# PANXIONG-CN/TEC-MoLLM

Hardware: AMD Instinct MI355X
Metric: train samples/sec (higher is better)
Workload: dtype f32; 1 GPU; BASELINE configs[1]: B=8/GPU, L_in=48, L_out=12, N=2911, F=10 (d_emb=12), 3 GPT-2 blocks, full fwd+bwd+AdamW, fp32, GATv2 per_timestep, dropout on (p=0.1); global_batch=8, parallelism=dp1, data_feed=fixed, launch=eager

## Files before the change

include/tecmollm.h:

```cpp
#ifndef TECMOLLM_H
#define TECMOLLM_H

#include <stdint.h>

#ifdef __cplusplus
extern "C" {
#endif

#define TECM_OK 0
#define TECM_E_ARG (-1)
#define TECM_E_ALIGN (-2)
#define TECM_E_LAUNCH (-3)
#define TECM_E_LDS (-4)

#define TECM_ABI_VERSION 17
int tecm_abi_version(void);
const char* tecm_last_error(void);

typedef struct TecmWin {
  int32_t enabled;
  int32_t N;
  int32_t Lin, Lout;
  int32_t stride_t;
  int32_t taps;
// ... 116 lines not shown
typedef struct TecmLnDyMap {
  int32_t T, N;
  TecmDrop drop;
} TecmLnDyMap;
int tecm_layernorm_bwd(const float* dy, int64_t lddy, const float* x, int64_t ldx, const float* gamma,
                       const float* stats, const float* dres, float* dx, void* dx_masked, int32_t masked_bf16,
                       const TecmDrop* mask_drop, float* dgb_partials, int32_t* num_blocks, int64_t M, int32_t D,
                       const TecmLnAdd* add ,
                       int32_t dy_bf16 ,
                       const TecmLnDyMap* dymap , void* stream);

#define TECM_ATT_OUT_BF16 1
#define TECM_ATT_QKV_BF16 2
#define TECM_ATT_DCTX_BF16 4
int tecm_attention_fwd(const float* qkv, void* ctx, int32_t io_bf16, int32_t B, int32_t T, int32_t N, int32_t heads,
                       int32_t D, const TecmDrop* prob_drop, void* stream);
int tecm_attention_bwd(const float* qkv, const float* dctx, void* dqkv, int32_t io_bf16, int32_t B, int32_t T, int32_t N,
                       int32_t heads, int32_t D, const TecmDrop* prob_drop, void* stream);

int tecm_colsum(const float* in, int64_t ld, int64_t outer, int64_t inner, int32_t nseg, int32_t C,
                float* out, int64_t ldo, int32_t accumulate, float scale, const TecmDrop* in_drop,
                float* workspace , void* stream);
int tecm_colsum_twin(const float* in, int64_t ld, int64_t outer, int64_t inner, int32_t nseg, int32_t C,
                     float* out, int64_t ldo, int32_t accumulate, float scale, const TecmDrop* in_drop,
                     float* workspace, void* twin_bf16, int64_t ld_twin, void* stream);

int tecm_huber_fwd_bwd(const float* pred, const float* target, float* dpred, float* loss_out,
                       int64_t n, float delta, float grad_scale, float* workspace ,
                       void* stream);

int tecm_conv_weight_pack(const float* w, float* fwd_pack, float* bwd_pack, int32_t Cout, int32_t Cin,
                          int32_t k, void* stream);
int tecm_conv_weight_unpack(const float* dpack, float* dw, int32_t Cout, int32_t Cin, int32_t k,
                            void* stream);

typedef struct TecmConvDx {
  const void* dy;
  const void* wpack;
  float* dinp;
  int32_t B, Lc, N, Cout, ld_in, _pad;
} TecmConvDx;
int tecm_conv_dx_pack(const float* w3, const float* w5, const float* w7, void* wpack, int32_t Cout, int32_t Cin,
                      int32_t ld_in, void* stream);
int tecm_conv_dx_bf16(const TecmConvDx* p, void* stream);
typedef struct TecmConvFwd {
  const void* inp;
  const void* wpack;
  const float* bias;
  float* y;
  int32_t B, Lc, N, Cout, ld_in, y_bf16;
  float* stats;
  float eps;
  int32_t _pad;
} TecmConvFwd;
int tecm_conv_fwd_pack(const float* w3, const float* w5, const float* w7, void* wpack, int32_t Cout, int32_t Cin,
                       int32_t ld_in, void* stream);
int tecm_conv_fwd_bf16(const TecmConvFwd* p, void* stream);
int tecm_conv_fwd_pack_f32(const float* w3, const float* w5, const float* w7, float* wpack, int32_t Cout, int32_t Cin,
                           int32_t ld_in, void* stream);
int tecm_conv_fwd_f32(const TecmConvFwd* p, void* stream);
int tecm_conv_dx_pack_f32(const float* w3, const float* w5, const float* w7, float* wpack, int32_t Cout, int32_t Cin,
                          int32_t ld_in, void* stream);
int tecm_conv_dx_f32(const TecmConvDx* p, void* stream);
int tecm_conv_fwd_supported(int32_t Lc, int32_t Cout, int32_t ld_in, int32_t f32);
int tecm_conv_dx_supported(int32_t Lc, int32_t Cout, int32_t ld_in, int32_t f32);

typedef struct TecmConvDw {
  const void* inp;
  const void* dy;
  float* workspace;
  float* dw3;
  float* dw5;
  float* dw7;
  int32_t B, Lc, N, Cout, Cin, ld_in, num_blocks, _pad;
} TecmConvDw;
int tecm_huber_fwd_bwd_strided(const float* pred, const int64_t* pred_strides , const float* target,
                               const int64_t* target_strides , float* dpred, float* loss_out, int32_t B, int32_t H,
                               int32_t N, float delta, float grad_scale, float* workspace , void* stream);

int64_t tecm_conv_dw_workspace(int32_t Cout, int32_t ld_in, int32_t num_blocks);
int tecm_conv_dw_bf16(const TecmConvDw* p, void* stream);
int tecm_conv_dw_f32(const TecmConvDw* p, void* stream);

int tecm_cast_bf16(const float* src, int64_t ld_src, void* dst, int64_t ld_dst, int64_t rows, int32_t cols, void* stream);

int tecm_weight_bf16(const float* src, int64_t ld_src, void* same_bf16, int64_t ld_same, void* transposed_bf16, int64_t ld_tr,
                     int32_t rows, int32_t cols, void* stream);

int tecm_dropout_apply(const float* src, int64_t ld_src, void* dst, int64_t ld_dst, int32_t dst_bf16, void* dst2_bf16,
                       int64_t ld_dst2, int64_t rows, int32_t cols, const TecmDrop* drop, void* stream);

int tecm_transpose_scale(const float* src, int64_t lds, float* dst, int64_t ldd, int32_t rows,
                         int32_t cols, float scale, void* stream);

int tecm_lora_fold(const float* lora_B, int32_t n_out, int32_t r, float scale, void* w_kn, int64_t ld_kn, int32_t kn_bf16,
                   void* w_nk, int64_t ld_nk, int32_t nk_bf16, int32_t k_off, void* stream);

int tecm_pack_vectors(const float* const* srcs, const int32_t* lens, int32_t count, float* dst, void* stream);

#define TECM_NORM_BLOCKS 512
typedef struct {
  int64_t n;
  float* param; float* grad; float* exp_avg; float* exp_avg_sq;
  double* partials;
  float* total_norm_out;
  float lr, beta1, beta2, eps, weight_decay, max_norm, grad_scale;
// ... 35 lines not shown
```

tec-mollm_amd/csrc/conv_seq.hip:

```cpp
#include "common.h"
#include <type_traits>

typedef float f32x16 __attribute__((ext_vector_type(16)));
typedef __bf16 bf16x8 __attribute__((ext_vector_type(8)));
typedef unsigned int u32x4 __attribute__((ext_vector_type(4)));
typedef float f32x4 __attribute__((ext_vector_type(4)));

namespace tecm_convseq {

#ifndef CDX_ABLATE
#define CDX_ABLATE 0
#endif

constexpr int NB = 4;
constexpr int NTH = 256;
constexpr int MAXT = 6;

__host__ __device__ __forceinline__ int seg_nact(int d) {
  const int a = d < 3 ? 3 - d : d - 3;
  return a <= 1 ? 3 : (a == 2 ? 2 : 1);
}

struct Args {
  const void* dy;
// ... 325 lines not shown
    while (k >= seg_nact(d) * Cout) {
      k -= seg_nact(d) * Cout;
      ++d;
    }
    const int col = (3 - seg_nact(d)) * Cout + k;
    const int j = col / Cout, co = col - j * Cout;
    const int kj = 3 + 2 * j, tau = (kj - 1) / 2 - (d - 3);
    const float* w = j == 0 ? w3 : (j == 1 ? w5 : w7);
    float v = 0.f;
    if (ci < Cin && tau >= 0 && tau < kj) v = w[((int64_t)co * Cin + ci) * kj + tau];
    wpack[i] = (__bf16)v;
  }
}

}

namespace tecm_convseq {

__device__ __forceinline__ float wave_total_dpp(float v) {
  auto step = [](float x, auto ctrl, auto rmask) {
    constexpr int C = decltype(ctrl)::value, R = decltype(rmask)::value;
    return x + __builtin_bit_cast(float, __builtin_amdgcn_update_dpp(0, __builtin_bit_cast(int, x), C, R, 0xF, false));
  };
  v = step(v, std::integral_constant<int, 0xB1>{}, std::integral_constant<int, 0xF>{});
  v = step(v, std::integral_constant<int, 0x4E>{}, std::integral_constant<int, 0xF>{});
  v = step(v, std::integral_constant<int, 0x141>{}, std::integral_constant<int, 0xF>{});
  v = step(v, std::integral_constant<int, 0x140>{}, std::integral_constant<int, 0xF>{});
  v = step(v, std::integral_constant<int, 0x142>{}, std::integral_constant<int, 0xA>{});
  v = step(v, std::integral_constant<int, 0x143>{}, std::integral_constant<int, 0xC>{});
  return __builtin_bit_cast(float, __builtin_amdgcn_readlane(__builtin_bit_cast(int, v), 63));
}

constexpr int FMAXU = 12;
#ifndef CFW_PD
#define CFW_PD 4
#endif
#ifndef CFW_ABLATE
#define CFW_ABLATE 0
#endif
#ifndef CFW_PD32
#define CFW_PD32 1
#endif
struct FArgs {
  const void* inp;
  const void* wpack;
  const float* bias;
  float* y;
  int y16;
  float* stats;
  float eps;
  int B, Lc, N, Cout, ld_in, TC, nchunk, nblk, pitch;
  int nb32;
  unsigned long long assign;
};

#ifdef CFW_STAMPS
__device__ unsigned long long cfw_stamps[16 * 8192];
}
extern "C" int tecm_cfw_stamps_read(unsigned long long* dst, int n) {
  return (int)hipMemcpyFromSymbol(dst, HIP_SYMBOL(tecm_convseq::cfw_stamps), sizeof(unsigned long long) * n);
}
namespace tecm_convseq {
#define CFW_STAMP(i) do { if (threadIdx.x == 0 && blockIdx.x < 8192) cfw_stamps[blockIdx.x * 16 + (i)] = __builtin_amdgcn_s_memrealtime(); } while (0)
#else
#define CFW_STAMP(i) do { } while (0)
#endif
__global__ __launch_bounds__(NTH, 3) void conv_fwd_seq_kernel(const FArgs a) {
  extern __shared__ __attribute__((aligned(16))) unsigned char lds[];
  CFW_STAMP(0);
  const int tid = threadIdx.x, lane = tid & 63;
  const int wave = __builtin_amdgcn_readfirstlane(tid >> 6);
  const int r = lane & 31, h = lane >> 5;
  int tile = blockIdx.x;
  const int nbk = tile % a.nblk;
  tile /= a.nblk;
  const int chunk = tile % a.nchunk, b = tile / a.nchunk;
  const int n0 = nbk * NB, t0 = chunk * a.TC;
  const int tc = min(a.TC, a.Lc - t0);
  const int steps = tc + 7;
  const int CT = 3 * a.Cout;

  {
    const int cpr = a.ld_in / 8;
    const int total = steps * NB * cpr;
    for (int idx = tid; idx < total; idx += NTH) {
      const int row = idx / cpr, ch = idx - row * cpr;
      const int ts = t0 - 3 + (row >> 2);
      const int ng = min(n0 + (row & 3), a.N - 1);
      u32x4 v = {0u, 0u, 0u, 0u};
      if (!(CFW_ABLATE & 1) && ts >= 0 && ts < a.Lc)
        v = *reinterpret_cast<const u32x4*>(static_cast<const __bf16*>(a.inp) + (((int64_t)b * a.Lc + ts) * a.N + ng) * a.ld_in + ch * 8);
      *reinterpret_cast<u32x4*>(lds + row * a.pitch + ch * 16) = v;
    }
  }
  __syncthreads();
  CFW_STAMP(1);

  const int ntt = tc >> 3;
  const int cpt = a.ld_in / 8;
  const unsigned cpt_magic = (unsigned)((65536 + cpt - 1) / cpt);
  __shared__ float xst[4][3][2 * NB + 1];
  if (a.stats && lane < 3) xst[wave][lane][0] = -1.f;
#pragma unroll 1
  for (int ui = 0; ui < 3; ++ui) {
    const int u = (int)((a.assign >> (12 * wave + 4 * ui)) & 15ull);
    if (u == 15) break;
// ... 97 lines not shown
              s1[e & 3] += dv;
              s2[e & 3] += dv * dv;
            }
          }
        const float ucnt = (float)(32 * tc);
#pragma unroll
        for (int n = 0; n < NB; ++n) {
          const float t1 = wave_total_dpp(s1[n]), t2 = wave_total_dpp(s2[n]);
          if (lane == 0) {
            xst[wave][ui][1 + n] = sh + t1 / ucnt;
            xst[wave][ui][1 + NB + n] = fmaxf(t2 - t1 * t1 / ucnt, 0.f);
          }
        }
        if (lane == 0) xst[wave][ui][0] = (float)j;
      }
      continue;
    }
    float* yb = a.y + (((int64_t)b * a.Lc + t0 + h) * a.N + n0) * CT + col0 + r;
#pragma unroll
    for (int i = 0; i < MAXT; ++i) {
      if (i < ntt) {
#pragma unroll
        for (int e = 0; e < 16; ++e) {
          const int n = e & 3;
          if (n0 + n < a.N) yb[(8 * i + 2 * (e >> 2)) * tstride + n * CT] = acc[i][e] + bv;
        }
      }
    }
  }
  CFW_STAMP(8);
  if (a.stats) {
    __syncthreads();
    if (tid < 3 * NB) {
      const int jb = tid / NB, n = tid % NB;
      const float ucnt = (float)(32 * tc);
      float cnt = 0.f, mean = 0.f, m2 = 0.f;
      for (int w = 0; w < 4; ++w)
        for (int q = 0; q < 3; ++q)
          if (xst[w][q][0] == (float)jb) {
            const float tot = cnt + ucnt, fr = ucnt / tot, dl = xst[w][q][1 + n] - mean;
            m2 += xst[w][q][1 + NB + n] + dl * dl * cnt * fr;
            mean += dl * fr;
            cnt = tot;
          }
      if (n0 + n < a.N) {
        float* st = a.stats + (((int64_t)b * a.N + n0 + n) * 3 + jb) * 2;
        st[0] = mean;
        st[1] = 1.0f / sqrtf(m2 / cnt + a.eps);
      }
    }
  }
}

__global__ __launch_bounds__(NTH, 2) void conv_fwd_seq_f32_kernel(const FArgs a) {
  extern __shared__ __attribute__((aligned(16))) unsigned char lds[];
  const int tid = threadIdx.x, lane = tid & 63;
  const int wave = __builtin_amdgcn_readfirstlane(tid >> 6);
  const int r = lane & 31, h = lane >> 5;
  int tile = blockIdx.x;
  const int nbk = tile % a.nblk;
  tile /= a.nblk;
  const int chunk = tile % a.nchunk, b = tile / a.nchunk;
  const int n0 = nbk * NB, t0 = chunk * a.TC;
  const int tc = min(a.TC, a.Lc - t0);
  const int steps = tc + 7;
  const int CT = 3 * a.Cout;
  {
    const int cpr = a.ld_in / 4;
    const int total = steps * NB * cpr;
    const float* src = static_cast<const float*>(a.inp);
    for (int idx = tid; idx < total; idx += NTH) {
      const int row = idx / cpr, ch = idx - row * cpr;
      const int ts = t0 - 3 + (row >> 2);
      const int ng = min(n0 + (row & 3), a.N - 1);
      u32x4 v = {0u, 0u, 0u, 0u};
      if (ts >= 0 && ts < a.Lc)
        v = *reinterpret_cast<const u32x4*>(src + (((int64_t)b * a.Lc + ts) * a.N + ng) * a.ld_in + ch * 4);
      *reinterpret_cast<u32x4*>(lds + row * a.pitch + ch * 16) = v;
    }
  }
  __syncthreads();

  const int ntt = tc >> 3;
  const int cpt = a.ld_in / 4;
  const unsigned cpt_magic = (unsigned)((65536 + cpt - 1) / cpt);
#pragma unroll 1
  for (int ui = 0; ui < 3; ++ui) {
    const int u = (int)((a.assign >> (12 * wave + 4 * ui)) & 15ull);
    if (u == 15) break;
    const int j = u / a.nb32, kb = u - j * a.nb32;
    const int pad = j + 1, col0 = j * a.Cout + 32 * kb;
    const int st3 = 3 * a.ld_in / 8, st5 = 5 * a.ld_in / 8, st7 = 7 * a.ld_in / 8;
    const int nsteps = j == 0 ? st3 : (j == 1 ? st5 : st7);
    const int woff = (j == 0 ? 0 : (j == 1 ? st3 : st3 + st5)) * a.nb32 + kb * nsteps;
    f32x16 acc[MAXT];
#pragma unroll
    for (int i = 0; i < MAXT; ++i)
#pragma unroll
      for (int e = 0; e < 16; ++e) acc[i][e] = 0.f;
    const f32x4* wp = reinterpret_cast<const f32x4*>(a.wpack) + (int64_t)woff * 64 + lane;
    auto kloop = [&](auto ntc) {
      constexpr int NTT = decltype(ntc)::value;
      auto rd = [&](int s, f32x4 (&df)[NTT]) {
        const int q = 2 * s + h;
        const int tap = (int)((q * cpt_magic) >> 16), c4 = q - tap * cpt;
        const int off0 = ((tap - pad + 3) * 4 + r) * a.pitch + c4 * 16;
#pragma unroll
        for (int i = 0; i < NTT; ++i) df[i] = *reinterpret_cast<const f32x4*>(lds + off0 + 32 * i * a.pitch);
      };
      f32x4 wq[CFW_PD32], df[NTT];
#pragma unroll
      for (int p_ = 0; p_ < CFW_PD32; ++p_) wq[p_] = wp[min(p_, nsteps - 1) * 64];
      rd(0, df);
      for (int s = 0; s < nsteps; ++s) {
        const int sn = min(s + 1, nsteps - 1);
        const f32x4 wn = wp[min(s + CFW_PD32, nsteps - 1) * 64];
        f32x4 dn[NTT];
        rd(sn, dn);
#pragma unroll
        for (int jj = 0; jj < 4; ++jj)
#pragma unroll
          for (int i = 0; i < NTT; ++i) acc[i] = __builtin_amdgcn_mfma_f32_32x32x2f32(df[i][jj], wq[0][jj], acc[i], 0, 0, 0);
#pragma unroll
        for (int p_ = 0; p_ + 1 < CFW_PD32; ++p_) wq[p_] = wq[p_ + 1];
        wq[CFW_PD32 - 1] = wn;
#pragma unroll
        for (int i = 0; i < NTT; ++i) df[i] = dn[i];
      }
    };
    switch (ntt) {
      case 1: kloop(std::integral_constant<int, 1>{}); break;
      case 2: kloop(std::integral_constant<int, 2>{}); break;
      case 3: kloop(std::integral_constant<int, 3>{}); break;
      case 4: kloop(std::integral_constant<int, 4>{}); break;
      case 5: kloop(std::integral_constant<int, 5>{}); break;
      default: kloop(std::integral_constant<int, MAXT>{}); break;
    }
    const float bv = a.bias[col0 + r];
    float* yb = a.y + (((int64_t)b * a.Lc + t0 + h) * a.N + n0) * CT + col0 + r;
    const int tstride = a.N * CT;
#pragma unroll
    for (int i = 0; i < MAXT; ++i) {
      if (i < ntt) {
#pragma unroll
        for (int e = 0; e < 16; ++e) {
          const int n = e & 3;
          if (n0 + n < a.N) yb[(8 * i + 2 * (e >> 2)) * tstride + n * CT] = acc[i][e] + bv;
        }
      }
    }
  }
}

__global__ __launch_bounds__(256) void conv_fwd_pack_f32_kernel(const float* __restrict__ w3, const float* __restrict__ w5,
                                                                const float* __restrict__ w7, float* __restrict__ wpack,
                                                                int Cout, int Cin, int ld_in) {
  const int nblk = Cout / 32;
  int steps[3], base[3], tot = 0;
  for (int j = 0; j < 3; ++j) {
    steps[j] = (3 + 2 * j) * ld_in / 8;
    base[j] = tot;
    tot += steps[j] * nblk;
  }
  const int total = tot * 256;
  for (int i = blockIdx.x * 256 + threadIdx.x; i < total; i += gridDim.x * 256) {
    const int jj = i & 3, lane = (i >> 2) & 63, f = i >> 8;
    int j = 2;
    if (f < base[1]) j = 0; else if (f < base[2]) j = 1;
    const int fl = f - base[j], blk = fl / steps[j], s = fl - blk * steps[j];
    const int k = 8 * s + 4 * (lane >> 5) + jj;
    const int tap = k / ld_in, ci = k - tap * ld_in, kj = 3 + 2 * j;
    const float* w = j == 0 ? w3 : (j == 1 ? w5 : w7);
    float v = 0.f;
    if (tap < kj && ci < Cin) v = w[((int64_t)(32 * blk + (lane & 31)) * Cin + ci) * kj + tap];
    wpack[i] = v;
  }
}

__global__ __launch_bounds__(256) void conv_fwd_pack_kernel(const float* __restrict__ w3, const float* __restrict__ w5,
                                                            const float* __restrict__ w7, __bf16* __restrict__ wpack,
                                                            int Cout, int Cin, int ld_in) {
  const int nblk = Cout / 32;
  int steps[3], base[3], tot = 0;
  for (int j = 0; j < 3; ++j) {
    steps[j] = ((3 + 2 * j) * ld_in + 15) / 16;
    base[j] = tot;
    tot += steps[j] * nblk;
  }
  const int total = tot * 512;
  for (int i = blockIdx.x * 256 + threadIdx.x; i < total; i += gridDim.x * 256) {
    const int e = i & 7, lane = (i >> 3) & 63, f = i >> 9;
    int j = 2;
    if (f < base[1]) j = 0; else if (f < base[2]) j = 1;
    const int fl = f - base[j], blk = fl / steps[j], s = fl - blk * steps[j];
    const int k = 16 * s + 8 * (lane >> 5) + e;
    const int tap = k / ld_in, ci = k - tap * ld_in, kj = 3 + 2 * j;
    const float* w = j == 0 ? w3 : (j == 1 ? w5 : w7);
    float v = 0.f;
    if (tap < kj && ci < Cin) v = w[((int64_t)(32 * blk + (lane & 31)) * Cin + ci) * kj + tap];
    wpack[i] = (__bf16)v;
// ... 5 lines not shown
extern "C" int tecm_conv_fwd_pack(const float* w3, const float* w5, const float* w7, void* wpack, int32_t Cout, int32_t Cin,
                                  int32_t ld_in, void* stream) {
  using namespace tecm_convseq;
  TECM_REQUIRE(w3 && w5 && w7 && wpack, TECM_E_ARG, "tecm_conv_fwd_pack: null pointer");
  TECM_REQUIRE(Cout > 0 && Cout % 32 == 0 && Cout <= 128 && Cin > 0 && Cin <= ld_in && ld_in % 8 == 0, TECM_E_ARG,
               "tecm_conv_fwd_pack: Cout a multiple of 32 up to 128, Cin <= ld_in, ld_in a multiple of 8");
  int tot = 0;
  for (int j = 0; j < 3; ++j) tot += (((3 + 2 * j) * ld_in + 15) / 16) * (Cout / 32);
  const int total = tot * 512;
  hipLaunchKernelGGL(conv_fwd_pack_kernel, dim3((total + 255) / 256), dim3(256), 0, (hipStream_t)stream, w3, w5, w7,
                     static_cast<__bf16*>(wpack), Cout, Cin, ld_in);
  TECM_CHECK_LAUNCH("tecm_conv_fwd_pack");
  return TECM_OK;
}

static size_t conv_fwd_lds(int Lc, int ld_in, bool f32, int* pitch_out, int* tc_out) {
  using namespace tecm_convseq;
  int slots = ld_in * (f32 ? 4 : 2) / 16;
  if (slots % 2 == 0) ++slots;
  const int pitch = slots * 16;
  const int TC = 8 * MAXT < Lc ? 8 * MAXT : Lc;
  if (pitch_out) *pitch_out = pitch;
  if (tc_out) *tc_out = TC;
  return (size_t)(TC + 7) * NB * pitch;
}

extern "C" int tecm_conv_fwd_supported(int32_t Lc, int32_t Cout, int32_t ld_in, int32_t f32) {
  if (Lc <= 0 || Lc % 8 != 0 || Cout <= 0 || Cout % 32 != 0 || Cout > 128 || ld_in <= 0 || ld_in % 8 != 0 || ld_in > 128) return 0;
  return conv_fwd_lds(Lc, ld_in, f32 != 0, nullptr, nullptr) <= 64 * 1024 ? 1 : 0;
}

static int conv_fwd_launch(const TecmConvFwd* p, void* stream, bool f32, const char* who) {
  using namespace tecm_convseq;
  TECM_REQUIRE(p && p->inp && p->wpack && p->bias && p->y, TECM_E_ARG, "%s: null pointer", who);
  TECM_REQUIRE(p->B > 0 && p->Lc > 0 && p->N > 0 && p->Lc % 8 == 0, TECM_E_ARG,
               "%s: bad shape (the sequence length must be a multiple of 8)", who);
  TECM_REQUIRE(p->Cout % 32 == 0 && p->Cout > 0 && p->Cout <= 128 && p->ld_in % 8 == 0 && p->ld_in > 0 && p->ld_in <= 128,
               TECM_E_ARG, "%s: Cout a multiple of 32 up to 128, ld_in a multiple of 8 up to 128", who);
  TECM_REQUIRE(tecm_aligned(p->inp, 16) && tecm_aligned(p->wpack, 16), TECM_E_ALIGN, "%s: 16-byte aligned pointers", who);
  FArgs a;
  a.inp = p->inp;
  a.wpack = p->wpack;
  a.bias = p->bias;
  a.y = p->y;
  a.y16 = p->y_bf16 != 0;
  a.stats = p->stats;
  a.eps = p->eps;
  TECM_REQUIRE(!(a.y16 && f32), TECM_E_ARG, "%s: a bf16 y is written by the bf16 kernel only", who);
  TECM_REQUIRE(!a.y16 || tecm_aligned(p->y, 4), TECM_E_ALIGN, "%s: y must be 4-byte aligned", who);
  a.B = p->B; a.Lc = p->Lc; a.N = p->N; a.Cout = p->Cout; a.ld_in = p->ld_in;
  const size_t lds = conv_fwd_lds(p->Lc, p->ld_in, f32, &a.pitch, &a.TC);
  a.nchunk = (p->Lc + a.TC - 1) / a.TC;
  a.nblk = (p->N + NB - 1) / NB;
  TECM_REQUIRE(!a.stats || (a.y16 && !f32 && a.nchunk == 1 && p->eps > 0.f), TECM_E_ARG,
               "%s: GroupNorm statistics come with a bf16 y and sequences of at most %d steps (one tile per sequence)", who, a.TC);
  TECM_REQUIRE(lds <= 64 * 1024, TECM_E_LDS, "%s: %zu B of LDS per tile", who, lds);
  const int nb32 = p->Cout / 32;
  a.nb32 = nb32;
  const int nunits = 3 * nb32;
  int load[4] = {0, 0, 0, 0}, cnt[4] = {0, 0, 0, 0};
  unsigned long long assign = ~0ull;
  for (int u = nunits - 1; u >= 0; --u) {
    const int j = u / nb32, st = f32 ? (3 + 2 * j) * p->ld_in / 8 : ((3 + 2 * j) * p->ld_in + 15) / 16;
    int best = -1;
    for (int w = 0; w < 4; ++w)
      if (cnt[w] < 3 && (best < 0 || load[w] < load[best])) best = w;
    TECM_REQUIRE(best >= 0, TECM_E_ARG, "%s: more than 12 (kernel size, channel block) units", who);
    const int sh = 12 * best + 4 * cnt[best]++;
    assign = (assign & ~(15ull << sh)) | ((unsigned long long)u << sh);
    load[best] += st;
  }
  a.assign = assign;
  const int64_t tiles = (int64_t)p->B * a.nchunk * a.nblk;
  TECM_REQUIRE(tiles < ((int64_t)1 << 31), TECM_E_ARG, "%s: too many tiles", who);
  if (f32) hipLaunchKernelGGL(conv_fwd_seq_f32_kernel, dim3((unsigned)tiles), dim3(NTH), lds, (hipStream_t)stream, a);
  else hipLaunchKernelGGL(conv_fwd_seq_kernel, dim3((unsigned)tiles), dim3(NTH), lds, (hipStream_t)stream, a);
  TECM_CHECK_LAUNCH("tecm_conv_fwd");
  return TECM_OK;
}

extern "C" int tecm_conv_fwd_bf16(const TecmConvFwd* p, void* stream) { return conv_fwd_launch(p, stream, false, "tecm_conv_fwd_bf16"); }
extern "C" int tecm_conv_fwd_f32(const TecmConvFwd* p, void* stream) { return conv_fwd_launch(p, stream, true, "tecm_conv_fwd_f32"); }

extern "C" int tecm_conv_fwd_pack_f32(const float* w3, const float* w5, const float* w7, float* wpack, int32_t Cout,
                                      int32_t Cin, int32_t ld_in, void* stream) {
  using namespace tecm_convseq;
  TECM_REQUIRE(w3 && w5 && w7 && wpack, TECM_E_ARG, "tecm_conv_fwd_pack_f32: null pointer");
  TECM_REQUIRE(Cout > 0 && Cout % 32 == 0 && Cout <= 128 && Cin > 0 && Cin <= ld_in && ld_in % 8 == 0, TECM_E_ARG,
               "tecm_conv_fwd_pack_f32: Cout a multiple of 32 up to 128, Cin <= ld_in, ld_in a multiple of 8");
  int tot = 0;
  for (int j = 0; j < 3; ++j) tot += ((3 + 2 * j) * ld_in / 8) * (Cout / 32);
  const int total = tot * 256;
  hipLaunchKernelGGL(conv_fwd_pack_f32_kernel, dim3((total + 255) / 256), dim3(256), 0, (hipStream_t)stream, w3, w5, w7, wpack,
                     Cout, Cin, ld_in);
  TECM_CHECK_LAUNCH("tecm_conv_fwd_pack_f32");
  return TECM_OK;
}

extern "C" int tecm_conv_dx_pack(const float* w3, const float* w5, const float* w7, void* wpack, int32_t Cout, int32_t Cin,
                                 int32_t ld_in, void* stream) {
  using namespace tecm_convseq;
  TECM_REQUIRE(w3 && w5 && w7 && wpack, TECM_E_ARG, "tecm_conv_dx_pack: null pointer");
  TECM_REQUIRE(Cout > 0 && Cout % 64 == 0 && Cin > 0 && Cin <= ld_in && ld_in % 4 == 0, TECM_E_ARG,
               "tecm_conv_dx_pack: Cout must be a multiple of 64, Cin <= ld_in, ld_in a multiple of 4");
  const int NCI = (ld_in + 31) / 32;
  const int total = 15 * Cout * NCI * 32;
  hipLaunchKernelGGL(conv_dx_pack_kernel, dim3((total + 255) / 256), dim3(256), 0, (hipStream_t)stream, w3, w5, w7,
                     static_cast<__bf16*>(wpack), Cout, Cin, NCI);
// ... 96 lines not shown
```

tec-mollm_amd/tecmollm/_lib.py:

```python
from __future__ import annotations

import ctypes as C
import os
from typing import Optional

import torch

_HERE = os.path.dirname(os.path.abspath(__file__))
LIB_PATH = os.environ.get("TECM_LIB", os.path.join(_HERE, "libtecmollm_hip.so"))
ABI_VERSION = 17

c_f32p = C.c_void_p


class TecmWin(C.Structure):
    _fields_ = [("enabled", C.c_int32), ("N", C.c_int32), ("Lin", C.c_int32), ("Lout", C.c_int32),
                ("stride_t", C.c_int32), ("taps", C.c_int32), ("Cw", C.c_int32), ("pad", C.c_int32)]


class TecmDrop(C.Structure):
    _fields_ = [("p", C.c_float), ("_pad", C.c_int32), ("seed", C.c_uint64), ("ld", C.c_int64), ("seed_dev", C.c_void_p)]


class TecmGemm(C.Structure):
# ... 51 lines not shown


class TecmLnDyMap(C.Structure):
    _fields_ = [("T", C.c_int32), ("N", C.c_int32), ("drop", TecmDrop)]


class TecmAdamW(C.Structure):
    _fields_ = [
        ("n", C.c_int64),
        ("param", c_f32p), ("grad", c_f32p), ("exp_avg", c_f32p), ("exp_avg_sq", c_f32p),
        ("partials", C.c_void_p), ("total_norm_out", c_f32p),
        ("lr", C.c_float), ("beta1", C.c_float), ("beta2", C.c_float), ("eps", C.c_float),
        ("weight_decay", C.c_float), ("max_norm", C.c_float), ("grad_scale", C.c_float),
        ("step", C.c_int32), ("zero_grad", C.c_int32), ("_pad", C.c_int32),
    ]


class TecmMetrics(C.Structure):
    _fields_ = [
        ("pred", c_f32p), ("p_stride_s", C.c_int64), ("p_stride_h", C.c_int64), ("p_stride_i", C.c_int64),
        ("target", c_f32p), ("t_stride_s", C.c_int64), ("t_stride_h", C.c_int64), ("t_stride_i", C.c_int64),
        ("S", C.c_int64), ("H", C.c_int32), ("_pad", C.c_int32), ("I", C.c_int64),
        ("mean", C.c_double), ("scale", C.c_double),
        ("clip_lo", C.c_float), ("clip_hi", C.c_float), ("clip", C.c_int32), ("_pad2", C.c_int32),
        ("stats", C.c_void_p),
    ]


class TecmWindowBatch(C.Structure):
    _fields_ = [
        ("X", c_f32p), ("TF", c_f32p), ("Y", c_f32p), ("starts", C.c_void_p), ("starts_host_check", C.c_void_p),
        ("T", C.c_int64), ("row", C.c_int64),
        ("N", C.c_int32), ("L_in", C.c_int32), ("L_out", C.c_int32), ("F_t", C.c_int32), ("B", C.c_int32),
        ("_pad", C.c_int32),
        ("x_out", c_f32p), ("tf_out", c_f32p), ("y_out", c_f32p),
    ]

class TecmConvDx(C.Structure):
    _fields_ = [("dy", C.c_void_p), ("wpack", C.c_void_p), ("dinp", c_f32p),
                ("B", C.c_int32), ("Lc", C.c_int32), ("N", C.c_int32), ("Cout", C.c_int32), ("ld_in", C.c_int32),
                ("_pad", C.c_int32)]


class TecmConvDw(C.Structure):
    _fields_ = [("inp", C.c_void_p), ("dy", C.c_void_p), ("workspace", c_f32p), ("dw3", c_f32p), ("dw5", c_f32p),
                ("dw7", c_f32p),
                ("B", C.c_int32), ("Lc", C.c_int32), ("N", C.c_int32), ("Cout", C.c_int32), ("Cin", C.c_int32),
                ("ld_in", C.c_int32), ("num_blocks", C.c_int32), ("_pad", C.c_int32)]


class TecmConvFwd(C.Structure):
    _fields_ = [("inp", C.c_void_p), ("wpack", C.c_void_p), ("bias", c_f32p), ("y", c_f32p),
                ("B", C.c_int32), ("Lc", C.c_int32), ("N", C.c_int32), ("Cout", C.c_int32), ("ld_in", C.c_int32),
                ("y_bf16", C.c_int32), ("stats", c_f32p), ("eps", C.c_float), ("_pad", C.c_int32)]


TECM_NORM_BLOCKS = 512
TECM_METRIC_STATS = 8


EXPORTS = {
    "tecm_abi_version": (C.c_int, []),
    "tecm_last_error": (C.c_char_p, []),
    "tecm_gemm_f32": (C.c_int, [C.POINTER(TecmGemm), C.c_void_p]),
    "tecm_gemm_bf16": (C.c_int, [C.POINTER(TecmGemm), C.c_void_p]),
    "tecm_gemm_bf16x3": (C.c_int, [C.POINTER(TecmGemm), C.c_void_p]),
    "tecm_gemm_bf16x6": (C.c_int, [C.POINTER(TecmGemm), C.c_void_p]),
    "tecm_spatial_fwd": (C.c_int, [C.POINTER(TecmSpatial), C.c_void_p]),
    "tecm_spatial_fwd2_ws_floats": (C.c_int64, [C.POINTER(TecmSpatial)]),
    "tecm_spatial_fwd2": (C.c_int, [C.POINTER(TecmSpatial), c_f32p, C.c_void_p]),
    "tecm_spatial_bwd": (C.c_int, [C.POINTER(TecmSpatial), C.POINTER(TecmSpatialGrads), C.c_void_p]),
    "tecm_spatial_bwd_blocks": (C.c_int, [C.POINTER(TecmSpatial)]),
    "tecm_spatial_bwd2_blocks": (C.c_int, [C.POINTER(TecmSpatial)]),
    "tecm_spatial_bwd2": (C.c_int, [C.POINTER(TecmSpatial), C.POINTER(TecmSpatialGrads), c_f32p, C.c_void_p]),
    "tecm_groupnorm_gelu_fwd": (C.c_int, [c_f32p, c_f32p, c_f32p, c_f32p, c_f32p, C.c_int32, C.c_int32, C.c_int32,
                                          C.c_int32, C.c_float, C.c_int32, C.c_int32, C.c_void_p]),
    "tecm_gn_y16_supported": (C.c_int, [C.c_int32, C.c_int32, C.c_int32]),
    "tecm_groupnorm_gelu_bwd": (C.c_int, [c_f32p, C.c_int32, c_f32p, c_f32p, c_f32p, c_f32p, c_f32p, c_f32p,
                                          C.POINTER(C.c_int32), C.c_int32, C.c_int32, C.c_int32, C.c_int32,
                                          C.c_int32, c_f32p, C.c_void_p]),
    "tecm_layernorm_fwd": (C.c_int, [c_f32p, C.c_int64, c_f32p, c_f32p, c_f32p, C.c_int64, C.c_void_p, C.c_int64,
                                     C.c_void_p, C.c_int64, C.POINTER(TecmDrop), C.c_int32, C.c_int32,
                                     c_f32p, C.c_int64, C.c_int32, C.c_float, C.c_void_p]),
    "tecm_layernorm_bwd": (C.c_int, [c_f32p, C.c_int64, c_f32p, C.c_int64, c_f32p, c_f32p, c_f32p, c_f32p, C.c_void_p,
                                     C.c_int32, C.POINTER(TecmDrop), c_f32p, C.POINTER(C.c_int32), C.c_int64, C.c_int32,
                                     C.POINTER(TecmLnAdd), C.c_int32, C.POINTER(TecmLnDyMap), C.c_void_p]),
    "tecm_attention_fwd": (C.c_int, [c_f32p, C.c_void_p, C.c_int32, C.c_int32, C.c_int32, C.c_int32, C.c_int32,
                                     C.c_int32, C.POINTER(TecmDrop), C.c_void_p]),
    "tecm_cast_bf16": (C.c_int, [c_f32p, C.c_int64, C.c_void_p, C.c_int64, C.c_int64, C.c_int32, C.c_void_p]),
    "tecm_attention_bwd": (C.c_int, [c_f32p, c_f32p, c_f32p, C.c_int32, C.c_int32, C.c_int32, C.c_int32, C.c_int32,
                                     C.c_int32, C.POINTER(TecmDrop), C.c_void_p]),
    "tecm_colsum": (C.c_int, [c_f32p, C.c_int64, C.c_int64, C.c_int64, C.c_int32, C.c_int32, c_f32p, C.c_int64,
                              C.c_int32, C.c_float, C.POINTER(TecmDrop), c_f32p, C.c_void_p]),
    "tecm_colsum_twin": (C.c_int, [c_f32p, C.c_int64, C.c_int64, C.c_int64, C.c_int32, C.c_int32, c_f32p, C.c_int64,
                                   C.c_int32, C.c_float, C.POINTER(TecmDrop), c_f32p, C.c_void_p, C.c_int64, C.c_void_p]),
    "tecm_huber_fwd_bwd": (C.c_int, [c_f32p, c_f32p, c_f32p, c_f32p, C.c_int64, C.c_float, C.c_float, c_f32p,
                                     C.c_void_p]),
    "tecm_huber_fwd_bwd_strided": (C.c_int, [c_f32p, C.POINTER(C.c_int64), c_f32p, C.POINTER(C.c_int64), c_f32p, c_f32p,
                                             C.c_int32, C.c_int32, C.c_int32, C.c_float, C.c_float, c_f32p, C.c_void_p]),
    "tecm_lora_fold": (C.c_int, [c_f32p, C.c_int32, C.c_int32, C.c_float, C.c_void_p, C.c_int64, C.c_int32, C.c_void_p,
                                 C.c_int64, C.c_int32, C.c_int32, C.c_void_p]),
    "tecm_pack_vectors": (C.c_int, [C.POINTER(C.c_void_p), C.POINTER(C.c_int32), C.c_int32, c_f32p, C.c_void_p]),
    "tecm_conv_weight_pack": (C.c_int, [c_f32p, c_f32p, c_f32p, C.c_int32, C.c_int32, C.c_int32, C.c_void_p]),
    "tecm_conv_weight_unpack": (C.c_int, [c_f32p, c_f32p, C.c_int32, C.c_int32, C.c_int32, C.c_void_p]),
    "tecm_conv_dx_pack": (C.c_int, [c_f32p, c_f32p, c_f32p, C.c_void_p, C.c_int32, C.c_int32, C.c_int32, C.c_void_p]),
    "tecm_conv_dx_bf16": (C.c_int, [C.POINTER(TecmConvDx), C.c_void_p]),
    "tecm_conv_fwd_pack": (C.c_int, [c_f32p, c_f32p, c_f32p, C.c_void_p, C.c_int32, C.c_int32, C.c_int32, C.c_void_p]),
# ... 72 lines not shown
```

tec-mollm_amd/tecmollm/functions.py:

```python
from __future__ import annotations

import os
from dataclasses import dataclass
import weakref
from typing import List, Optional

import torch

from . import devcheck, ops
from ._lib import TecmSpatial, TecmSpatialGrads, check, lib, stream_ptr
from .graph import GraphMeta
from .ops import (A_KM, A_MK, ACT_GELU_ERF, ACT_GELU_TANH, B_KN, B_NK, colsum, drop, gemm, pick_split_k, win)

PRE16 = os.environ.get("TECM_PRE16", "1")[:1] != "0"
GRAD16 = os.environ.get("TECM_GRAD16", "1")[:1] != "0"
QKV16 = os.environ.get("TECM_QKV16", "1")[:1] != "0"

import ctypes as C

CP = 24
C_FEAT = 22
LORA_R = 32
LORA_SCALE = 2.0
GPT_HEADS = 12
# ... 233 lines not shown
        g.src_ptr, g.src_col, g.src_ptr_off = meta.src_ptr.data_ptr(), meta.src_col.data_ptr(), meta.src_ptr_off.data_ptr()
        check(lib().tecm_spatial_bwd(C.byref(d), C.byref(g), stream_ptr()), "tecm_spatial_bwd(GAT only)")
        s = colsum(partials, pld, nblocks, 1, 1, pld)[0]
        o = 0
        dWl = s[o:o + Cc * Cc].view(Cc, Cc); o += Cc * Cc
        dbl = s[o:o + Cc]; o += Cc
        dWr = s[o:o + Cc * Cc].view(Cc, Cc); o += Cc * Cc
        dbr = s[o:o + Cc]; o += Cc
        datt = s[o:o + Cc].view_as(att)
        dbias = colsum(dpad, CP, G * N, 1, 1, CP)[0, :Cc]
        return (None, dWl, dbl, dWr, dbr, datt, dbias, None, None, None, None)


def conv_block_acts16(Lc: int, N: int, Cout: int) -> bool:
    return Cout >= 64 and ops.gn_reg_ok(Lc, N, Cout)


def conv_block_y16(Lc: int, N: int, Cout: int, ld_in: int) -> bool:
    CT = 3 * Cout
    return (conv_block_acts16(Lc, N, Cout) and ld_in % 8 == 0 and ops.conv_fwd_seq_ok(Lc, Cout, ld_in, f32=False)
            and ops.gn_y16_ok(Lc, N, Cout) and ops.uses_bf16(CT, Cout, Cout, CT, b_layout=B_KN))


def conv_storage_policy(N: int):
    def policy(L: int, Cout: int, Cin: int):
        ld_in = CP if Cin == C_FEAT else Cin
        return conv_block_acts16(L, N, Cout), conv_block_y16(L, N, Cout, ld_in)
    return policy


class ConvBlockFn(torch.autograd.Function):

    @staticmethod
    def forward(ctx, inp, inp16, cin: int, stride: int, need_dinp: bool, bf16: bool,
                w3, b3, g3, be3, w5, b5, g5, be5, w7, b7, g7, be7, wf, bf):
        B, Lc, N, ld_in = inp.shape
        Cout = w3.shape[0]
        CT = 3 * Cout
        M = B * Lc * N
        ws = (w3, w5, w7)
        bs = (b3, b5, b7)
        r16 = int(bf16) == ops.PREC_BF16 and conv_block_acts16(Lc, N, Cout)
        adt = torch.bfloat16 if r16 else torch.float32
        side16 = r16
        packs = []
        seq_in = inp16 if (side16 and inp16 is not None) else (inp if int(bf16) == ops.PREC_FP32 else None)
        fwd_seq = seq_in is not None and ops.conv_fwd_seq_ok(Lc, Cout, ld_in, f32=seq_in.dtype == torch.float32)
        y16 = r16 and fwd_seq and seq_in.dtype == torch.bfloat16 and conv_block_y16(Lc, N, Cout, ld_in)
        y = torch.empty(B, Lc, N, CT, device=inp.device, dtype=torch.bfloat16 if y16 else torch.float32)
        bgb = ops.pack_vectors([b3, b5, b7, g3, g5, g7, be3, be5, be7])
        bias3, gamma, beta = bgb[:CT], bgb[CT:2 * CT], bgb[2 * CT:]
        stats = _empty(B * N, 3, 2, like=inp)
        st_given = y16 and ops.conv_fwd_stats_ok(Lc)
        if fwd_seq:
            ops.conv_fwd(seq_in.detach(), w3.detach(), w5.detach(), w7.detach(), bias3, y, B, Lc, N, Cout, cin, ld_in,
                         stats=stats if st_given else None)
        dx_gemm = need_dinp and not ConvBlockFn._dx_seq(bf16, r16, Lc, Cout, ld_in)
        for j, (w, b) in enumerate(zip(ws, bs)):
            k = w.shape[2]
            if fwd_seq and not dx_gemm:
                packs.append(w.new_empty(0))
                continue
            wp = w if ld_in == cin else torch.nn.functional.pad(w, (0, 0, 0, ld_in - cin))
            fp, bp = ops.conv_weight_pack(wp.contiguous(), want_bwd=True)
            packs.append(bp)
            if fwd_seq:
                continue
            a_in = inp16 if (inp16 is not None and side16 and ld_in % 8 == 0) else inp
            gemm(M, Cout, k * ld_in, a_in, ld_in, fp, k * ld_in, y, CT, c_off=j * Cout,
                 a_win=win(N, Lc, Lc, 1, k, ld_in, (k - 1) // 2), bias=b, bf16=bf16)
        Lo = (Lc - 1) // stride + 1
        compact = stride > 1 and ops.gn_reg_ok(Lc, N, Cout) and int(bf16) in (ops.PREC_FP32, ops.PREC_BF16)
        La = Lo if compact else Lc
        act = torch.empty(B, La, N, CT, device=inp.device, dtype=adt)
        ops.groupnorm_gelu_fwd(y, gamma, beta, act, stats, B, Lc, N, Cout, act_stride=stride if compact else 1,
                               stats_given=st_given)
        out = _empty(B, Lo, N, Cout, like=inp)
        wf2 = wf.view(Cout, CT)
        out16 = None
        awin = None if compact else win(N, Lc, Lo, stride, 1, CT, 0)
        wfT16 = None
        if int(bf16) == ops.PREC_BF16 and compact and act.dtype == torch.bfloat16 and Cout % 8 == 0:
            wf2, wfT16 = ops.weight_bf16(wf2, same=True, transposed=True)
        ctx.wfT16 = wfT16
        if side16:
            out16 = torch.empty(B, Lo, N, Cout, device=inp.device, dtype=torch.bfloat16)
            gemm(B * Lo * N, Cout, CT, act, CT, wf2, CT, out16, Cout, a_win=awin, bias=bf, preact=(out, Cout), bf16=bf16)
            ctx.mark_non_differentiable(out16)
        else:
            gemm(B * Lo * N, Cout, CT, act, CT, wf2, CT, out, Cout, a_win=awin, bias=bf, bf16=bf16)
        ctx.save_for_backward(inp, y, act, stats, gamma, beta, wf, *packs)
        ctx.w357 = (w3.detach(), w5.detach(), w7.detach())
        ctx.inp16 = inp16 if (side16 and inp16 is not None and ld_in % 8 == 0) else None
        ctx.dims = (B, Lc, N, ld_in, cin, Cout, stride, Lo, need_dinp, bf16)
        ctx.compact = compact
        return out, out16

    @staticmethod
    def _dx_seq(bf16, dy16: bool, Lc: int, Cout: int, ld_in: int) -> bool:
        return int(bf16) in (ops.PREC_FP32, ops.PREC_BF16) and (dy16 or int(bf16) == ops.PREC_FP32) \
            and ops.conv_dx_seq_ok(Lc, Cout, ld_in, f32=not dy16)

    @staticmethod
    def backward(ctx, dout, _dout16=None):
        inp, y, act, stats, gamma, beta, wf, bp3, bp5, bp7 = ctx.saved_tensors
        B, Lc, N, ld_in, cin, Cout, stride, Lo, need_dinp, bf16 = ctx.dims
        CT = 3 * Cout
        M = B * Lc * N
        Mo = B * Lo * N
        dout = dout.contiguous()
        wf2 = wf.view(Cout, CT)
        if int(bf16) == ops.PREC_BF16 and act.dtype == torch.bfloat16 and ctx.compact and ops.tn_ok(Cout, CT, Mo) and Cout % 8 == 0:
            dout_g = torch.empty(Mo, Cout, device=dout.device, dtype=torch.bfloat16)
            dbf = colsum(dout, Cout, Mo, 1, 1, Cout, twin=dout_g)[0]
        else:
            dout_g = dout
            dbf = colsum(dout, Cout, Mo, 1, 1, Cout)[0]
        dwf = _empty(Cout, CT, like=inp)
        gemm(Cout, CT, Mo, dout_g, Cout, act, CT, dwf, CT, a_layout=A_KM, b_layout=B_KN,
             b_win=None if ctx.compact else win(N, Lc, Lo, stride, 1, CT, 0),
             split_k=pick_split_k(Cout, CT, Mo, prec=bf16), bf16=bf16)
        d16 = act.dtype == torch.bfloat16 and ops.uses_bf16(CT, Cout, Cout, CT, b_layout=B_KN)
        dact = torch.empty(B, Lo, N, CT, device=inp.device, dtype=torch.bfloat16 if d16 else torch.float32)
        if ctx.wfT16 is not None and dout_g.dtype == torch.bfloat16 and d16:
            gemm(Mo, CT, Cout, dout_g, Cout, ctx.wfT16, Cout, dact, CT, bf16=bf16)
        else:
            gemm(Mo, CT, Cout, dout_g, Cout, wf2, CT, dact, CT, b_layout=B_KN, bf16=bf16)
        dy = torch.empty(B, Lc, N, CT, device=inp.device, dtype=act.dtype)
        dgamma, dbeta, dbconv = ops.groupnorm_gelu_bwd(dact, stride, y, gamma, beta, stats, dy, B, Lc, N, Cout)
# ... 468 lines not shown
```

tec-mollm_amd/tecmollm/ops.py:

```python
from __future__ import annotations

import os
import ctypes as C
from typing import Optional, Tuple

import torch

from . import _lib
from ._lib import TecmDrop, TecmGemm, TecmWin, check, lib, ptr, stream_ptr

A_MK, A_KM = 0, 1
B_NK, B_KN = 0, 1
ACT_NONE, ACT_GELU_ERF, ACT_GELU_TANH = 0, 1, 2

_MASK64 = (1 << 64) - 1


def splitmix64(x: int) -> int:
    x = (x + 0x9E3779B97F4A7C15) & _MASK64
    z = x
    z = ((z ^ (z >> 30)) * 0xBF58476D1CE4E5B9) & _MASK64
    z = ((z ^ (z >> 27)) * 0x94D049BB133111EB) & _MASK64
    return z ^ (z >> 31)

# ... 566 lines not shown
    _timing.append((name, 2.0 * B * Lc * N * ld_in * 15 * Cout, e0, e1))


conv_dx_bf16 = conv_dx


def conv_dw_seq_ok(Lc: int, Cout: int, ld_in: int) -> bool:
    return (Lc % 4 == 0 and Lc > 0 and Cout in (64, 128) and ld_in in (24, 64)
            and os.environ.get("TECM_CONV_DW_SEQ", "1")[:1] != "0")


_cu_count = {}


def conv_dw(inp: torch.Tensor, dy: torch.Tensor, B: int, Lc: int, N: int, Cout: int, cin: int, ld_in: int):
    if inp.dtype != dy.dtype or dy.dtype not in (torch.bfloat16, torch.float32):
        raise _lib.TecmError("conv_dw: inp and dy are both bf16 or both fp32 tensors")
    f32 = dy.dtype == torch.float32
    run, what = (lib().tecm_conv_dw_f32, "tecm_conv_dw_f32") if f32 else (lib().tecm_conv_dw_bf16, "tecm_conv_dw_bf16")
    dev = dy.device
    nb = _cu_count.get(dev.index)
    if nb is None:
        nb = _cu_count[dev.index] = int(os.environ.get("TECM_CONV_DW_BLOCKS", 0)) or \
            torch.cuda.get_device_properties(dev).multi_processor_count
    nws = lib().tecm_conv_dw_workspace(Cout, ld_in, nb)
    if nws <= 0:
        raise _lib.TecmError(f"conv_dw: no kernel for Cout={Cout}, ld_in={ld_in}")
    ws = torch.empty(nws, device=dev, dtype=torch.float32)
    dws = [torch.empty(Cout, cin, k, device=dev, dtype=torch.float32) for k in (3, 5, 7)]
    d = _lib.TecmConvDw(inp=inp.data_ptr(), dy=dy.data_ptr(), workspace=ws.data_ptr(), dw3=dws[0].data_ptr(),
                        dw5=dws[1].data_ptr(), dw7=dws[2].data_ptr(), B=B, Lc=Lc, N=N, Cout=Cout, Cin=cin, ld_in=ld_in,
                        num_blocks=nb)
    if _timing is None:
        check(run(C.byref(d), stream_ptr()), what)
        return dws
    e0, e1 = torch.cuda.Event(enable_timing=True), torch.cuda.Event(enable_timing=True)
    e0.record()
    check(run(C.byref(d), stream_ptr()), what)
    e1.record()
    name = ("conv_dw_seq_f32_kernel" if f32 else "conv_dw_seq_kernel") + (f" M={15 * ld_in} N={Cout} K={B * Lc * N}" if _timing_detail else "")
    _timing.append((name, 2.0 * B * Lc * N * ld_in * 15 * Cout, e0, e1))
    return dws


def conv_fwd_seq_ok(Lc: int, Cout: int, ld_in: int, f32: bool = False) -> bool:
    return (os.environ.get("TECM_CONV_SEQ", "1")[:1] != "0" and os.environ.get("TECM_CONV_FWD_SEQ", "1")[:1] != "0"
            and lib().tecm_conv_fwd_supported(Lc, Cout, ld_in, 1 if f32 else 0) == 1)


def conv_fwd_stats_ok(Lc: int) -> bool:
    return Lc <= 48 and os.environ.get("TECM_CONV_STATS", "1")[:1] != "0"


def conv_fwd(inp: torch.Tensor, w3: torch.Tensor, w5: torch.Tensor, w7: torch.Tensor, bias: torch.Tensor,
             y: torch.Tensor, B: int, Lc: int, N: int, Cout: int, cin: int, ld_in: int,
             stats: Optional[torch.Tensor] = None, eps: float = 1e-5) -> None:
    if inp.dtype not in (torch.bfloat16, torch.float32) or y.dtype not in (torch.bfloat16, torch.float32) or \
            (y.dtype == torch.bfloat16 and inp.dtype != torch.bfloat16):
        raise _lib.TecmError("conv_fwd: inp is bf16 or fp32, y fp32 (or bf16 next to a bf16 inp)")
    f32 = inp.dtype == torch.float32
    if f32:
        nval = sum(((3 + 2 * j) * ld_in // 8) * (Cout // 32) for j in range(3)) * 256
        pack, run, what = lib().tecm_conv_fwd_pack_f32, lib().tecm_conv_fwd_f32, "tecm_conv_fwd_f32"
    else:
        nval = sum((((3 + 2 * j) * ld_in + 15) // 16) * (Cout // 32) for j in range(3)) * 512
        pack, run, what = lib().tecm_conv_fwd_pack, lib().tecm_conv_fwd_bf16, "tecm_conv_fwd_bf16"
    wpack = torch.empty(nval, device=y.device, dtype=inp.dtype)
    check(pack(w3.data_ptr(), w5.data_ptr(), w7.data_ptr(), wpack.data_ptr(), Cout, cin, ld_in, stream_ptr()), what + "/pack")
    d = _lib.TecmConvFwd(inp=inp.data_ptr(), wpack=wpack.data_ptr(), bias=bias.data_ptr(), y=y.data_ptr(), B=B, Lc=Lc,
                         N=N, Cout=Cout, ld_in=ld_in, y_bf16=1 if y.dtype == torch.bfloat16 else 0,
                         stats=ptr(stats), eps=eps)
    if _timing is None:
        check(run(C.byref(d), stream_ptr()), what)
        return
    e0, e1 = torch.cuda.Event(enable_timing=True), torch.cuda.Event(enable_timing=True)
    e0.record()
    check(run(C.byref(d), stream_ptr()), what)
    e1.record()
    name = ("conv_fwd_seq_f32_kernel" if f32 else "conv_fwd_seq_kernel") + \
        (f" M={B * Lc * N} N={3 * Cout} K={5 * ld_in}(avg)" if _timing_detail else "")
    _timing.append((name, 2.0 * B * Lc * N * Cout * 15 * ld_in, e0, e1))


conv_fwd_bf16 = conv_fwd


def transpose_scale(src: torch.Tensor, lds: int, dst: torch.Tensor, ldd: int, rows: int, cols: int, scale: float,
                    dst_off: int = 0) -> None:
    check(lib().tecm_transpose_scale(src.data_ptr(), lds, _off(dst, dst_off), ldd, rows, cols, scale, stream_ptr()),
          "tecm_transpose_scale")
```

Baseline: 126.0 samples/s.

## Fuse GroupNorm statistics and GELU activation into fp32 sequence conv forward

Extends the fp32 sequence conv forward kernel to compute per-group GroupNorm statistics from its register accumulators. After a block-level reduction it applies normalisation, gamma/beta and GELU, writing the strided activation tensor directly. This removes the separate groupnorm_gelu_fwd launch and its extra read of y for the fp32 path. It also raises launch_bounds occupancy from 2 to 4, which may pressure registers, and the fused epilogue re-reads y from global memory, relying on same-block writes being visible after __syncthreads.

```diff
diff --git a/include/tecmollm.h b/include/tecmollm.h
--- a/include/tecmollm.h
+++ b/include/tecmollm.h
@@ -192,6 +192,10 @@
   float* stats;
   float eps;
   int32_t _pad;
+  float* act;
+  const float* gamma;
+  const float* beta;
+  int32_t act_stride, _pad2;
 } TecmConvFwd;
 int tecm_conv_fwd_pack(const float* w3, const float* w5, const float* w7, void* wpack, int32_t Cout, int32_t Cin,
                        int32_t ld_in, void* stream);
diff --git a/tec-mollm_amd/csrc/conv_seq.hip b/tec-mollm_amd/csrc/conv_seq.hip
--- a/tec-mollm_amd/csrc/conv_seq.hip
+++ b/tec-mollm_amd/csrc/conv_seq.hip
@@ -401,6 +401,10 @@
   int B, Lc, N, Cout, ld_in, TC, nchunk, nblk, pitch;
   int nb32;
   unsigned long long assign;
+  float* act;
+  const float* gamma;
+  const float* beta;
+  int act_stride;
 };
 
 #ifdef CFW_STAMPS
@@ -604,7 +608,7 @@
   }
 }
 
-__global__ __launch_bounds__(NTH, 2) void conv_fwd_seq_f32_kernel(const FArgs a) {
+__global__ __launch_bounds__(NTH, 4) void conv_fwd_seq_f32_kernel(const FArgs a) {
   extern __shared__ __attribute__((aligned(16))) unsigned char lds[];
   const int tid = threadIdx.x, lane = tid & 63;
   const int wave = __builtin_amdgcn_readfirstlane(tid >> 6);
@@ -636,6 +640,8 @@
   const int ntt = tc >> 3;
   const int cpt = a.ld_in / 4;
   const unsigned cpt_magic = (unsigned)((65536 + cpt - 1) / cpt);
+  __shared__ float xst[4][3][2 * NB + 1];
+  if (a.stats && lane < 3) xst[wave][lane][0] = -1.f;
 #pragma unroll 1
   for (int ui = 0; ui < 3; ++ui) {
     const int u = (int)((a.assign >> (12 * wave + 4 * ui)) & 15ull);
@@ -697,7 +703,92 @@
 #pragma unroll
         for (int e = 0; e < 16; ++e) {
           const int n = e & 3;
-          if (n0 + n < a.N) yb[(8 * i + 2 * (e >> 2)) * tstride + n * CT] = acc[i][e] + bv;
+          acc[i][e] += bv;
+          if (n0 + n < a.N) yb[(8 * i + 2 * (e >> 2)) * tstride + n * CT] = acc[i][e];
+        }
+      }
+    }
+    if (a.stats) {
+      const float sh = __builtin_bit_cast(float, __builtin_amdgcn_readfirstlane(__builtin_bit_cast(int, acc[0][0])));
+      const float ucnt = (float)(32 * tc);
+#pragma unroll
+      for (int n = 0; n < NB; ++n) {
+        float s1 = 0.f, s2 = 0.f;
+#pragma unroll
+        for (int i = 0; i < MAXT; ++i)
+          if (i < ntt) {
+#pragma unroll
+            for (int e = n; e < 16; e += NB) {
+              const float dv = acc[i][e] - sh;
+              s1 += dv;
+              s2 += dv * dv;
+            }
+          }
+        const float t1 = wave_total_dpp(s1), t2 = wave_total_dpp(s2);
+        if (lane == 0) {
+          xst[wave][ui][1 + n] = sh + t1 / ucnt;
+          xst[wave][ui][1 + NB + n] = fmaxf(t2 - t1 * t1 / ucnt, 0.f);
+        }
+      }
+      if (lane == 0) xst[wave][ui][0] = (float)j;
+    }
+  }
+  if (!a.stats) return;
+  __shared__ float gst[3][NB][2];
+  __syncthreads();
+  if (tid < 3 * NB) {
+    const int jb = tid / NB, n = tid % NB;
+    const float ucnt = (float)(32 * tc);
+    float cnt = 0.f, mean = 0.f, m2 = 0.f;
+    for (int w = 0; w < 4; ++w)
+      for (int q = 0; q < 3; ++q)
+        if (xst[w][q][0] == (float)jb) {
+          const float tot = cnt + ucnt, fr = ucnt / tot, dl = xst[w][q][1 + n] - mean;
+          m2 += xst[w][q][1 + NB + n] + dl * dl * cnt * fr;
+          mean += dl * fr;
+          cnt = tot;
+        }
+    const float rstd = 1.0f / sqrtf(m2 / cnt + a.eps);
+    gst[jb][n][0] = mean;
+    gst[jb][n][1] = rstd;
+    if (n0 + n < a.N) {
+      float* st = a.stats + (((int64_t)b * a.N + n0 + n) * 3 + jb) * 2;
+      st[0] = mean;
+      st[1] = rstd;
+    }
+  }
+  if (!a.act) return;
+  __syncthreads();
+  {
+    const int QPR = CT / 4, S = a.act_stride;
+    const int La = (tc + S - 1) / S;
+    const int total = La * NB * QPR;
+    const float* ys = a.y + ((int64_t)b * a.Lc * a.N + n0) * CT;
+    float* as = a.act + ((int64_t)b * La * a.N + n0) * CT;
+    constexpr int AB = 6;
+    for (int i0 = tid; i0 < total; i0 += AB * NTH) {
+      float4 v[AB];
+#pragma unroll
+      for (int k = 0; k < AB; ++k) {
+        const int idx = min(i0 + k * NTH, total - 1);
+        const int q = idx % QPR, rn = idx / QPR, n = rn & (NB - 1), ta = rn >> 2;
+        const int nc = min(n, a.N - 1 - n0);
+        v[k] = *reinterpret_cast<const float4*>(ys + ((int64_t)ta * S * a.N + nc) * CT + 4 * q);
+      }
+#pragma unroll
+      for (int k = 0; k < AB; ++k) {
+        const int idx = i0 + k * NTH;
+        const int q = idx % QPR, rn = idx / QPR, n = rn & (NB - 1), ta = rn >> 2;
+        if (idx < total && n0 + n < a.N) {
+          const int c = 4 * q, jb = c / a.Cout;
+          const float mean = gst[jb][n][0], rstd = gst[jb][n][1];
+          const float4 g = *reinterpret_cast<const float4*>(a.gamma + c), be = *reinterpret_cast<const float4*>(a.beta + c);
+          float4 o;
+          o.x = gelu_erf_fast((v[k].x - mean) * rstd * g.x + be.x);
+          o.y = gelu_erf_fast((v[k].y - mean) * rstd * g.y + be.y);
+          o.z = gelu_erf_fast((v[k].z - mean) * rstd * g.z + be.z);
+          o.w = gelu_erf_fast((v[k].w - mean) * rstd * g.w + be.w);
+          *reinterpret_cast<float4*>(as + ((int64_t)ta * a.N + n) * CT + c) = o;
         }
       }
     }
@@ -809,8 +900,17 @@
   const size_t lds = conv_fwd_lds(p->Lc, p->ld_in, f32, &a.pitch, &a.TC);
   a.nchunk = (p->Lc + a.TC - 1) / a.TC;
   a.nblk = (p->N + NB - 1) / NB;
-  TECM_REQUIRE(!a.stats || (a.y16 && !f32 && a.nchunk == 1 && p->eps > 0.f), TECM_E_ARG,
-               "%s: GroupNorm statistics come with a bf16 y and sequences of at most %d steps (one tile per sequence)", who, a.TC);
+  TECM_REQUIRE(!a.stats || ((a.y16 || f32) && a.nchunk == 1 && p->eps > 0.f), TECM_E_ARG,
+               "%s: GroupNorm statistics come with a bf16 y (bf16 kernel) or the fp32 kernel, and sequences of at most %d steps "
+               "(one tile per sequence)", who, a.TC);
+  a.act = p->act;
+  a.gamma = p->gamma;
+  a.beta = p->beta;
+  a.act_stride = p->act_stride;
+  TECM_REQUIRE(!a.act || (f32 && a.stats && p->gamma && p->beta && p->act_stride >= 1), TECM_E_ARG,
+               "%s: the fused GroupNorm + GELU (act) needs the fp32 kernel, stats, gamma, beta and act_stride >= 1", who);
+  TECM_REQUIRE(!a.act || (tecm_aligned(p->act, 16) && tecm_aligned(p->y, 16) && tecm_aligned(p->gamma, 16) &&
+                          tecm_aligned(p->beta, 16)), TECM_E_ALIGN, "%s: act, y, gamma and beta must be 16-byte aligned", who);
   TECM_REQUIRE(lds <= 64 * 1024, TECM_E_LDS, "%s: %zu B of LDS per tile", who, lds);
   const int nb32 = p->Cout / 32;
   a.nb32 = nb32;
diff --git a/tec-mollm_amd/tecmollm/_lib.py b/tec-mollm_amd/tecmollm/_lib.py
--- a/tec-mollm_amd/tecmollm/_lib.py
+++ b/tec-mollm_amd/tecmollm/_lib.py
@@ -127,7 +127,8 @@
 class TecmConvFwd(C.Structure):
     _fields_ = [("inp", C.c_void_p), ("wpack", C.c_void_p), ("bias", c_f32p), ("y", c_f32p),
                 ("B", C.c_int32), ("Lc", C.c_int32), ("N", C.c_int32), ("Cout", C.c_int32), ("ld_in", C.c_int32),
-                ("y_bf16", C.c_int32), ("stats", c_f32p), ("eps", C.c_float), ("_pad", C.c_int32)]
+                ("y_bf16", C.c_int32), ("stats", c_f32p), ("eps", C.c_float), ("_pad", C.c_int32),
+                ("act", c_f32p), ("gamma", c_f32p), ("beta", c_f32p), ("act_stride", C.c_int32), ("_pad2", C.c_int32)]
 
 
 TECM_NORM_BLOCKS = 512
diff --git a/tec-mollm_amd/tecmollm/functions.py b/tec-mollm_amd/tecmollm/functions.py
--- a/tec-mollm_amd/tecmollm/functions.py
+++ b/tec-mollm_amd/tecmollm/functions.py
@@ -309,9 +309,16 @@
         bias3, gamma, beta = bgb[:CT], bgb[CT:2 * CT], bgb[2 * CT:]
         stats = _empty(B * N, 3, 2, like=inp)
         st_given = y16 and ops.conv_fwd_stats_ok(Lc)
+        Lo = (Lc - 1) // stride + 1
+        compact = stride > 1 and ops.gn_reg_ok(Lc, N, Cout) and int(bf16) in (ops.PREC_FP32, ops.PREC_BF16)
+        La = Lo if compact else Lc
+        act = torch.empty(B, La, N, CT, device=inp.device, dtype=adt)
+        gn_fused = (fwd_seq and seq_in.dtype == torch.float32 and not y16 and ops.conv_fwd_gn_ok(Lc)
+                    and act.dtype == torch.float32)
         if fwd_seq:
             ops.conv_fwd(seq_in.detach(), w3.detach(), w5.detach(), w7.detach(), bias3, y, B, Lc, N, Cout, cin, ld_in,
-                         stats=stats if st_given else None)
+                         stats=stats if (st_given or gn_fused) else None,
+                         act=act if gn_fused else None, gamma=gamma, beta=beta, act_stride=stride if compact else 1)
         dx_gemm = need_dinp and not ConvBlockFn._dx_seq(bf16, r16, Lc, Cout, ld_in)
         for j, (w, b) in enumerate(zip(ws, bs)):
             k = w.shape[2]
@@ -326,12 +333,9 @@
             a_in = inp16 if (inp16 is not None and side16 and ld_in % 8 == 0) else inp
             gemm(M, Cout, k * ld_in, a_in, ld_in, fp, k * ld_in, y, CT, c_off=j * Cout,
                  a_win=win(N, Lc, Lc, 1, k, ld_in, (k - 1) // 2), bias=b, bf16=bf16)
-        Lo = (Lc - 1) // stride + 1
-        compact = stride > 1 and ops.gn_reg_ok(Lc, N, Cout) and int(bf16) in (ops.PREC_FP32, ops.PREC_BF16)
-        La = Lo if compact else Lc
-        act = torch.empty(B, La, N, CT, device=inp.device, dtype=adt)
-        ops.groupnorm_gelu_fwd(y, gamma, beta, act, stats, B, Lc, N, Cout, act_stride=stride if compact else 1,
-                               stats_given=st_given)
+        if not gn_fused:
+            ops.groupnorm_gelu_fwd(y, gamma, beta, act, stats, B, Lc, N, Cout, act_stride=stride if compact else 1,
+                                   stats_given=st_given)
         out = _empty(B, Lo, N, Cout, like=inp)
         wf2 = wf.view(Cout, CT)
         out16 = None
diff --git a/tec-mollm_amd/tecmollm/ops.py b/tec-mollm_amd/tecmollm/ops.py
--- a/tec-mollm_amd/tecmollm/ops.py
+++ b/tec-mollm_amd/tecmollm/ops.py
@@ -642,13 +642,23 @@
     return Lc <= 48 and os.environ.get("TECM_CONV_STATS", "1")[:1] != "0"
 
 
+def conv_fwd_gn_ok(Lc: int) -> bool:
+    return conv_fwd_stats_ok(Lc) and os.environ.get("TECM_CONV_GN", "1")[:1] != "0"
+
+
 def conv_fwd(inp: torch.Tensor, w3: torch.Tensor, w5: torch.Tensor, w7: torch.Tensor, bias: torch.Tensor,
              y: torch.Tensor, B: int, Lc: int, N: int, Cout: int, cin: int, ld_in: int,
-             stats: Optional[torch.Tensor] = None, eps: float = 1e-5) -> None:
+             stats: Optional[torch.Tensor] = None, eps: float = 1e-5, act: Optional[torch.Tensor] = None,
+             gamma: Optional[torch.Tensor] = None, beta: Optional[torch.Tensor] = None, act_stride: int = 1) -> None:
     if inp.dtype not in (torch.bfloat16, torch.float32) or y.dtype not in (torch.bfloat16, torch.float32) or \
             (y.dtype == torch.bfloat16 and inp.dtype != torch.bfloat16):
         raise _lib.TecmError("conv_fwd: inp is bf16 or fp32, y fp32 (or bf16 next to a bf16 inp)")
     f32 = inp.dtype == torch.float32
+    if act is not None:
+        La = (Lc + act_stride - 1) // act_stride
+        if not f32 or stats is None or gamma is None or beta is None or act.dtype != torch.float32 or \
+                act.numel() != B * La * N * 3 * Cout:
+            raise _lib.TecmError(f"conv_fwd: act is the fp32 (B, {La}, N, 3*Cout) tensor of an fp32 input, with stats, gamma, beta")
     if f32:
         nval = sum(((3 + 2 * j) * ld_in // 8) * (Cout // 32) for j in range(3)) * 256
         pack, run, what = lib().tecm_conv_fwd_pack_f32, lib().tecm_conv_fwd_f32, "tecm_conv_fwd_f32"
@@ -659,7 +669,8 @@
     check(pack(w3.data_ptr(), w5.data_ptr(), w7.data_ptr(), wpack.data_ptr(), Cout, cin, ld_in, stream_ptr()), what + "/pack")
     d = _lib.TecmConvFwd(inp=inp.data_ptr(), wpack=wpack.data_ptr(), bias=bias.data_ptr(), y=y.data_ptr(), B=B, Lc=Lc,
                          N=N, Cout=Cout, ld_in=ld_in, y_bf16=1 if y.dtype == torch.bfloat16 else 0,
-                         stats=ptr(stats), eps=eps)
+                         stats=ptr(stats), eps=eps,
+                         act=ptr(act), gamma=ptr(gamma), beta=ptr(beta), act_stride=act_stride)
     if _timing is None:
         check(run(C.byref(d), stream_ptr()), what)
         return
```

Measured after the change: 126.7 samples/s (median of 6 runs). About the same (+0.5%).
